# tgsstdio/BirdNest.Audio

Hardware: AMD Instinct MI355X
Metric: decoded PCM MSamples/s/GPU (bit-exact) + achieved HBM GB/s vs roofline (higher is better)
Workload: dtype int32; 1 GPU; C2: 1024-frame batches, 44.1 kHz/16-bit stereo, bs 4096, LPC-8, Rice partition order 4 -> FLACDecoder 16-bit LE interleaved PCM; frames_per_batch=1024, compressed_bytes_per_batch=10724000, pcm_bytes_per_batch=16777216, parallelism=corpus of 1 x 1024 batches partitioned per rank (shard.partition) x1

## Files before the change

birdnest/audio_amd/csrc/bnflac_kernels.hip:

```cpp
#include <hip/hip_runtime.h>
#include <stdint.h>
#include <stdlib.h>
#include <atomic>
#include <mutex>
#include <type_traits>

#include "bnflac_device.h"

#define DEV __device__ __forceinline__

__constant__ uint8_t g_crc8_tab[256];
__constant__ uint16_t g_crc16_tab[8][256];
__constant__ uint16_t g_crc16_xpow[40];
__device__ unsigned long long g_stats[16];
DEV uint64_t tnow(bool on) {
#ifndef BNFLAC_PHASE_TIMERS
    (void)on;
    return 0ull;
#endif
    if (!on) return 0ull;
    const uint64_t t = __builtin_amdgcn_s_memtime();
    asm volatile("s_waitcnt lgkmcnt(0)" ::: "memory");
    return t;
}
#define STAT(on, i) do { if (on) { if (__builtin_amdgcn_read_exec() && (threadIdx.x & 63) == (uint32_t)__builtin_ctzll(__builtin_amdgcn_read_exec())) atomicAdd(&g_stats[i], 1ull); } } while (0)

typedef __attribute__((address_space(3))) uint32_t lds_u32;
typedef __attribute__((address_space(3))) uint16_t lds_u16;
typedef __attribute__((address_space(3))) void lds_void;
typedef uint32_t u32x4 __attribute__((ext_vector_type(4)));
typedef __attribute__((address_space(3))) u32x4 lds_u32x4;
DEV void lds_st128(const void *a, u32x4 v) {
    asm volatile("ds_write_b128 %0, %1" ::"v"((uint32_t)(uintptr_t)a), "v"(v) : "memory");
}
DEV u32x4 lds_ld128(const void *a) {
    u32x4 v;
    asm volatile("ds_read_b128 %0, %1" : "=v"(v) : "v"((uint32_t)(uintptr_t)a) : "memory");
    return v;
}
DEV void lds_st128(const lds_u32x4 *a, u32x4 v) {
    asm volatile("ds_write_b128 %0, %1" ::"v"((uint32_t)(uintptr_t)a), "v"(v) : "memory");
}
DEV u32x4 lds_ld128(const lds_u32x4 *a) {
    u32x4 v;
    asm volatile("ds_read_b128 %0, %1" : "=v"(v) : "v"((uint32_t)(uintptr_t)a) : "memory");
    return v;
}
DEV void lds_st64(const void *a, uint64_t v) {
    asm volatile("ds_write_b64 %0, %1" ::"v"((uint32_t)(uintptr_t)a), "v"(v) : "memory");
}
DEV uint64_t lds_ld64(const void *a) {
    uint64_t v;
    asm volatile("ds_read_b64 %0, %1" : "=v"(v) : "v"((uint32_t)(uintptr_t)a) : "memory");
    return v;
}
typedef __attribute__((address_space(1))) const void gvoid;
DEV void gst128(uint64_t addr, u32x4 v) { *(__attribute__((address_space(1))) u32x4 *)addr = v; }

#define BNF_MODE_WREDO 0x4000u
#define BNF_MODE_SW 0x8000u
#define BNF_ABLATE_NO_SW 0x10000u
#define BNF_MODE_LIST 0x20000u
#define BNF_MODE_SEG 0x80000000u
#define BNF_MODE_NOST 0x40000u
#define BNF_MODE_STREDO 0x80000u
#define BNF_ABLATE_NO_W8SPLIT 0x100000u

#define RING_MAX 16
#define RING_LANE_DW 256

struct BR {
    const uint32_t *__restrict__ w;
    uint32_t nw;
    uint32_t nblk;
    lds_u32 *ring;
    lds_u32 *lring;
    uint32_t rdepth, wmask;
    uint32_t wi, s, hi, lo, nx;
    uint32_t vendw, iend;
    uint32_t iend_old;
    uint32_t ra, vlim;
    bool stats;
};

DEV void br_init(BR &b, const uint32_t *words, uint64_t nbytes, lds_u32 *ring, uint32_t lane, uint32_t rdepth) {
    b.rdepth = rdepth;
    b.wmask = 4u * rdepth - 1u;
    b.w = words;
    b.nblk = (uint32_t)((nbytes + 15u) >> 4);
    b.nw = b.nblk * 4u;
    b.ring = ring;
    b.lring = ring + lane * 4u;
    b.wi = 2;
    b.s = b.hi = b.lo = b.nx = 0;
    b.vendw = b.iend = 0;
    b.iend_old = 0;
    b.stats = false;
}

DEV void wait_vm() { asm volatile("s_waitcnt vmcnt(0)" ::: "memory"); }
template <int N> DEV void wait_vm_but() { asm volatile("s_waitcnt vmcnt(%0)" ::"i"(N) : "memory"); }
DEV void wait_vm_n(uint32_t n) {
    switch (__builtin_amdgcn_readfirstlane(min(n, 63u))) {
#define WVN(k) case k: asm volatile("s_waitcnt vmcnt(" #k ")" ::: "memory"); break;
#define WVN8(k) WVN(k) WVN(k + 1) WVN(k + 2) WVN(k + 3) WVN(k + 4) WVN(k + 5) WVN(k + 6) WVN(k + 7)
        WVN8(0) WVN8(8) WVN8(16) WVN8(24) WVN8(32) WVN8(40) WVN8(48) WVN8(56)
#undef WVN8
#undef WVN
    default: break;
    }
}
DEV void lds_sync() { asm volatile("s_waitcnt lgkmcnt(0)" ::: "memory"); }

DEV uint32_t gword(const BR &b, uint32_t w) { return (w < b.nw) ? b.w[w] : 0u; }
DEV uint32_t ring_off(const BR &b, uint32_t w) {
    return ((w & (b.wmask & ~3u)) << 6) + (w & 3u);
}
DEV uint32_t ring_word(const BR &b, uint32_t w) { return b.lring[ring_off(b, w)]; }
#define LDS_DMA_ALIGN __attribute__((aligned(1024)))
// ... 519 lines not shown

DEV uint32_t st_hmask(uint32_t h, uint32_t o) {
    return h <= o ? ~0u : (h >= o + 4u ? 0u : (~0u << (8u * (h - o))));
}
struct CrcZ {
    uint32_t r0, r1, px;
};
DEV void crcz_w(CrcZ &c, uint32_t le) {
    const uint32_t W = __builtin_bswap32(le);
    const uint32_t H = __builtin_amdgcn_alignbit(c.r1, c.r0, 28);
    const uint32_t n0 = W ^ H ^ (H << 4);
    c.r1 = c.r0 ^ (H >> 28);
    c.r0 = n0;
}
DEV void crcz_blk(CrcZ &c, uint4 v) {
    c.px ^= v.x ^ v.y ^ v.z ^ v.w;
    crcz_w(c, v.x);
    crcz_w(c, v.y);
    crcz_w(c, v.z);
    crcz_w(c, v.w);
}
struct CrcP {
    uint32_t s[15];
    uint32_t px;
    uint32_t wc;
};
DEV void crcp_init(CrcP &c) {
#pragma unroll
    for (int k = 0; k < 15; k++) c.s[k] = 0u;
    c.px = 0u;
    c.wc = ~0u;
}
DEV void crcp_fold(CrcP &c, const u32x4 (&v)[4]) {
    const uint32_t W[16] = {v[0].x, v[0].y, v[0].z, v[0].w, v[1].x, v[1].y, v[1].z, v[1].w,
                            v[2].x, v[2].y, v[2].z, v[2].w, v[3].x, v[3].y, v[3].z, v[3].w};
    c.px ^= W[0] ^ W[1] ^ W[2] ^ W[3] ^ W[4] ^ W[5] ^ W[6] ^ W[7] ^ W[8] ^ W[9] ^ W[10] ^ W[11] ^ W[12] ^ W[13] ^
            W[14] ^ W[15];
    const uint32_t r0 = c.s[13] ^ c.s[14] ^ W[15] ^ W[0], r1 = c.s[0] ^ c.s[13] ^ W[14] ^ W[0],
                   r2 = c.s[0] ^ c.s[1] ^ c.s[14] ^ W[13];
#pragma unroll
    for (int d = 14; d >= 3; d--) c.s[d] = c.s[d - 2] ^ c.s[d - 1] ^ W[15 - d];
    c.s[2] = r2;
    c.s[1] = r1;
    c.s[0] = r0;
    c.wc++;
}
DEV CrcZ crcp_z(const CrcP &c) {
    CrcZ z{0u, 0u, 0u};
#pragma unroll
    for (int k = 14; k >= 0; k--) crcz_w(z, c.s[k]);
    z.px = c.px;
    return z;
}
template <bool ALL = false, class C>
DEV void crcp_hook(C &c, const BR &b, uint32_t lane, uint32_t cl) {
    for (uint32_t it = 0; any_lane(c.wc < cl) && (ALL || it == 0u); it++) {
        if (c.wc < cl) {
            const uint32_t L = c.wc;
            u32x4 v[4];
            if (L + 2u >= (b.iend >> 2)) {
#pragma unroll
                for (uint32_t i = 0; i < 4; i++)
                    v[i] = lds_ld128((const lds_u32x4 *)(b.ring + (((L & 1u) * 4u + i) * RING_LANE_DW) + lane * 4u));
                lds_sync();
                crcp_fold(c, v);
            } else {
                const u32x4 *g = (const u32x4 *)((const uint8_t *)b.w + (uint64_t)L * 64u);
#pragma unroll
                for (uint32_t i = 0; i < 4; i++) v[i] = g[i];
                crcp_fold(c, v);
            }
        }
    }
}

#define CRC_LINES 4

DEV uint32_t byte_keep(int32_t lo, int32_t hi, int32_t w) {
    const int32_t a = min(max(lo - 4 * w, 0), 4), b = min(max(hi - 4 * w, 0), 4);
    const uint32_t mlo = a >= 4 ? 0u : (0xFFFFFFFFu << (8 * a));
    const uint32_t mhi = b >= 4 ? 0xFFFFFFFFu : ((1u << (8 * b)) - 1u);
    return mlo & mhi;
}
DEV bool crcz_zero(const CrcZ &c) {
    if (__builtin_popcount(c.px) & 1) return false;
    uint64_t v = ((uint64_t)(c.r1 & 0x0FFFFFFFu) << 32) | c.r0;
#pragma unroll
    for (int i = 0; i < 4; i++) {
        const uint64_t h = v >> 15;
        v = (v & 0x7FFFu) ^ h ^ (h << 1);
    }
    return v == 0;
}
DEV void crcz_line(CrcZ &c, uint4 (&v)[4], uint32_t h) {
    if (h) {
#pragma unroll
        for (int u = 0; u < 4; u++) {
            v[u].x &= st_hmask(h, 16u * u);
            v[u].y &= st_hmask(h, 16u * u + 4u);
            v[u].z &= st_hmask(h, 16u * u + 8u);
            v[u].w &= st_hmask(h, 16u * u + 12u);
        }
    }
#pragma unroll
    for (int u = 0; u < 4; u++) crcz_blk(c, v[u]);
}
template <int NL = CRC_LINES>
DEV bool st_crc16_ok(const uint8_t *__restrict__ bytes, uint64_t b0, uint64_t b1, CrcZ c = CrcZ{0u, 0u, 0u},
                     uint64_t from = 0) {
    const uint64_t p0 = max(b0 & ~(uint64_t)63u, from);
    const uint32_t h = p0 < b0 ? (uint32_t)(b0 & 63u) : 0u;
    const uint32_t nl = b1 > p0 ? (uint32_t)((b1 - p0) >> 6) : 0u;
    uint64_t p = p0;
    if (nl) {
        const uint4 *q = (const uint4 *)(bytes + p0);
        uint4 buf[NL][4];
#pragma unroll
        for (int d = 0; d < NL; d++)
#pragma unroll
            for (int u = 0; u < 4; u++) buf[d][u] = q[4u * min((uint32_t)d, nl - 1u) + u];
#pragma unroll
        for (int u = 0; u < 4; u++) {
// ... 590 lines not shown
    uint32_t incl = c;
    const uint32_t lane = threadIdx.x & 63;
    for (int o = 1; o < 64; o <<= 1) {
        uint32_t y = __shfl_up(incl, o);
        if (lane >= (unsigned)o) incl += y;
    }
    if (lane == 63) wtot[threadIdx.x >> 6] = incl;
    __syncthreads();
    uint32_t wpre = 0;
    for (uint32_t wv = 0; wv < (threadIdx.x >> 6); wv++) wpre += wtot[wv];
    uint32_t pos = block_offs[blockIdx.x] + wpre + incl - c;
    for (int i = 0; i < SCAN_BYTES_PER_THREAD; i++) {
        if (is_sync(d, n, base + i)) {
            if (pos < cap) out[pos] = base + i;
            pos++;
        }
    }
}

#define PARSE_RD 8
static_assert(PARSE_RD == 8, "pk_ra and the walk's pair steps (slot masks 0x3F3 / 0x1C0C, slot bits 10-12) assume an 8-slot ring");
template <int CPM>
DEV void parse_frame(const uint32_t *__restrict__ words, uint64_t nbytes, const uint64_t *__restrict__ frame_offs,
                     uint32_t nframes, const bnf_stream_params &sp, const uint64_t *__restrict__ out_sample_in,
                     uint64_t base_sample, bnf_frame_info *__restrict__ info, uint32_t ablate, lds_u32 *ring,
                     uint32_t f, uint32_t *__restrict__ crcp) {
    if (f >= nframes) return;
    bnf_frame_info fi;
    fi.status = BNF_ST_OK;
    fi.err = -1;
    fi.frame_off = frame_offs[f];
    fi.resume_bit = 0;
    fi.cached = -1;
    fi.blocksize = fi.sample_rate = fi.channels = fi.assignment = fi.bps = 0;
    fi.number_type = 0;
    fi.unparseable = 0;
    fi.number = 0;
    fi.out_sample = 0;
    fi.crc8 = fi.crc16_calc = fi.crc16_read = fi.crc_ok = 0;
    fi.flags = 0;
    fi.reserved = 0;
    uint32_t ss[8];
#pragma unroll
    for (int c = 0; c < 8; c++) ss[c] = 0;
    const uint64_t limit = nbytes * 8u;
    const uint64_t fbit = fi.frame_off * 8u;
    BR b;
    br_init(b, words, nbytes, ring, threadIdx.x, PARSE_RD);
    CrcP cp;
    crcp_init(cp);
    uint32_t st = parse_header(b, fbit, limit, sp, fi);
    if (st == BNF_ST_ERROR && br_pos(b) > limit) st = BNF_ST_TRUNC;
    if (CPM && crcp != nullptr && st == BNF_ST_OK && fi.channels == 2u && !(ablate & 16u)) {
        const uint32_t h = (uint32_t)(fi.frame_off & 63u);
        const u32x4 *g = (const u32x4 *)((const uint8_t *)words + (fi.frame_off & ~(uint64_t)63u));
        u32x4 v[4];
#pragma unroll
        for (uint32_t i = 0; i < 4; i++) {
            v[i] = g[i];
            v[i].x &= st_hmask(h, 16u * i);
            v[i].y &= st_hmask(h, 16u * i + 4u);
            v[i].z &= st_hmask(h, 16u * i + 8u);
            v[i].w &= st_hmask(h, 16u * i + 12u);
        }
        cp.wc = (uint32_t)(fi.frame_off >> 6);
        crcp_fold(cp, v);
    }
    if (st == BNF_ST_OK) {
        uint64_t sample;
        if (fi.number_type == 1) sample = fi.number;
        else if (sp.has_stream_info && sp.min_blocksize == sp.max_blocksize) sample = (uint64_t)sp.min_blocksize * fi.number;
        else sample = (uint64_t)fi.blocksize * fi.number;
        fi.out_sample = out_sample_in ? out_sample_in[f] : sample - base_sample;
        uint32_t maxorder = 0;
        bool raw = false;
        for (uint32_t ch = 0; ch < fi.channels; ch++) {
            const uint32_t here = (uint32_t)(br_pos(b) - fbit);
#pragma unroll
            for (int c = 0; c < 8; c++) ss[c] = (uint32_t)c == ch ? here : ss[c];
            if (ch + 1 == fi.channels) {
                const uint32_t x = br_peek(b) >> 24;
                if (!(x & 0x80u) && (x & 0x7Eu) >= 0x40u) maxorder = max(maxorder, ((x >> 1) & 31u) + 1u);
                raw = raw || (x & 0x7Eu) < 4u;
                break;
            }
            if (ablate & 16u) {
#pragma unroll
                for (int c = 0; c < 8; c++) ss[c] = (uint32_t)c == ch + 1 ? here : ss[c];
                continue;
            }
            SubHdr h;
            int32_t err = -1;
            uint32_t bps = sub_bps(fi, ch);
            st = parse_subframe_head<false>(b, bps, fi.blocksize, limit, h, nullptr, nullptr, err);
            if (st == BNF_ST_OK) {
                if (h.type == T_LPC) maxorder = max(maxorder, h.order);
                raw = raw || h.type == T_CONST || h.type == T_VERB;
                if (!(h.type == T_FIXED || h.type == T_LPC) || h.order > (fi.bps > 16u ? 12u : 8u)) cp.wc = ~0u;
                if (h.type == T_VERB) br_skip(b, (uint64_t)h.bps * fi.blocksize);
                else if (h.type == T_FIXED || h.type == T_LPC) st = skip_residual<CPM != 0>(b, h, fi.blocksize, limit, ablate, cp);
                if (st == BNF_ST_OK && br_pos(b) > limit) st = BNF_ST_TRUNC;
            }
            if (st == BNF_ST_ERROR && br_pos(b) > limit) st = BNF_ST_TRUNC;
            if (st != BNF_ST_OK) {
                if (st == BNF_ST_ERROR) {
                    fi.err = err;
                    fi.resume_bit = br_pos(b);
                }
                break;
            }
        }
        if (maxorder > 16) fi.flags |= BNF_FL_W32;
        else if (maxorder > 8 || (maxorder > 0 && fi.bps > 16)) fi.flags |= BNF_FL_W16;
        else if (fi.channels == 2 && fi.bps <= 16 && !raw) fi.flags |= BNF_FL_ST;
        if (maxorder > 0 && maxorder <= 12 && fi.channels == 2 && fi.bps > 16 && fi.bps <= 24 && !raw) fi.flags |= BNF_FL_SW;
    }
    fi.status = st;
#pragma unroll
// ... 1201 lines not shown
            if ((threadIdx.x & 63) >= (unsigned)o) incl += y;
        }
        if ((threadIdx.x & 63) == 63) wsum[threadIdx.x >> 6] = incl;
        __syncthreads();
        if (threadIdx.x == 0)
            for (int w = 1; w < 16; w++) wsum[w] += wsum[w - 1];
        __syncthreads();
        const uint64_t wprefix = (threadIdx.x >= 64) ? wsum[(threadIdx.x >> 6) - 1] : 0ull;
        if (i < n) v[i] = carry + wprefix + incl - x;
        __syncthreads();
        if (threadIdx.x == 1023) carry += wprefix + incl;
        __syncthreads();
    }
    if (threadIdx.x == 0) *total = carry;
}

__global__ void __launch_bounds__(256) k_chain_emit(const uint64_t *__restrict__ cand, uint32_t ncand,
                                                    const bnf_frame_info *__restrict__ info,
                                                    const uint32_t *__restrict__ mark, const uint32_t *__restrict__ pos,
                                                    const uint64_t *__restrict__ out_sample, bnf_stream_params sp,
                                                    uint64_t *__restrict__ d_offs, uint64_t *__restrict__ d_os,
                                                    bnf_frame_info *__restrict__ d_info, uint32_t cap,
                                                    uint32_t *__restrict__ nframes) {
    const uint32_t i = blockIdx.x * 256u + threadIdx.x;
    if (i >= ncand || !mark[i]) return;
    const uint32_t p = pos[i];
    if (p >= cap) return;
    const uint64_t os = out_sample[p];
    if (sp.has_stream_info && sp.total_samples > 0 && os >= sp.total_samples) {
        atomicMin(nframes, p);
        return;
    }
    d_offs[p] = cand[i];
    if (d_os) d_os[p] = os;
    if (d_info) {
        bnf_frame_info fi = info[i];
        fi.out_sample = os;
        d_info[p] = fi;
    }
}
#endif

#if BNF_TU == 3 || BNF_TU == 4 || BNF_TU == 7
#define ST_CHK 16
#define ST2_CHK 32
#define ST_RD 8

struct StCh {
    BR b;
    uint32_t cp[4];
    uint32_t q[8];
    int32_t sh;
    uint32_t k, km, k1, k32;
    uint32_t esc, left, pidx, nparts, psamples, plen, pesc, porder, order;
    uint32_t wasted;
    int32_t lim, mx, mn;
};

DEV uint32_t st_pk(int32_t lo, int32_t hi) { return __builtin_amdgcn_perm((uint32_t)hi, (uint32_t)lo, 0x05040100u); }
typedef short st_s2 __attribute__((ext_vector_type(2)));
DEV int32_t st_d2(uint32_t a, uint32_t b, int32_t acc) {
    return __builtin_amdgcn_sdot2(__builtin_bit_cast(st_s2, a), __builtin_bit_cast(st_s2, b), acc, false);
}
DEV int32_t st_d2z(uint32_t a, uint32_t b) {
    int32_t r;
    asm("v_dot2_i32_i16 %0, %1, %2, 0" : "=v"(r) : "v"(a), "v"(b));
    return r;
}

DEV bool st_setup(StCh &z, uint32_t bps, uint32_t bs, uint64_t limit) {
    SubHdr h;
    int32_t warm[8], coef[8], err = -1;
    const uint32_t st = parse_subframe_head<true, 8>(z.b, bps, bs, limit, h, warm, coef, err);
    if (st != BNF_ST_OK) return false;
    if (h.type != T_FIXED && h.type != T_LPC) return false;
    if (h.type == T_LPC && (h.order > 8 || h.path == P_WIDE)) return false;
    if (h.bps > 17) return false;
    int32_t c[8], w[8];
    bool in16 = true;
#pragma unroll
    for (int t = 0; t < 8; t++) {
        c[t] = 0;
        w[t] = ((uint32_t)t < h.order) ? warm[t] : 0;
        in16 = in16 && w[t] >= -32768 && w[t] <= 32767;
    }
    if (!in16) return false;
    z.sh = 0;
    z.lim = 0x7FFF;
    if (h.type == T_LPC) {
#pragma unroll
        for (int t = 0; t < 8; t++) c[t] = ((uint32_t)t < h.order) ? coef[t] : 0;
        if (h.path == P_MMX16) z.sh = ((uint32_t)h.shift >= 32u) ? 31 : h.shift;
        else z.sh = h.shift & 31;
    } else {
        const uint32_t o = h.order;
        c[0] = o == 1 ? 1 : o == 2 ? 2 : o == 3 ? 3 : o == 4 ? 4 : 0;
        c[1] = o == 2 ? -1 : o == 3 ? -3 : o == 4 ? -6 : 0;
        c[2] = o == 3 ? 1 : o == 4 ? 4 : 0;
        c[3] = o == 4 ? -1 : 0;
    }
#pragma unroll
    for (int k = 0; k < 4; k++) z.cp[k] = st_pk(c[2 * k], c[2 * k + 1]);
#pragma unroll
    for (int t = 0; t < 8; t++) z.q[t] = st_pk(w[t], t ? w[t - 1] : 0);
    z.order = h.order;
    z.wasted = h.wasted;
    z.porder = h.porder;
    z.nparts = 1u << h.porder;
    z.psamples = h.porder ? bs >> h.porder : bs - h.order;
    z.plen = h.rice2 ? 5u : 4u;
    z.pesc = h.rice2 ? 31u : 15u;
    z.left = 0;
    z.pidx = 0;
    z.esc = 0;
    z.k = 0;
    z.km = 31;
    z.k1 = 1;
    z.k32 = 32;
    z.mx = 0;
    z.mn = 0;
    return true;
}

template <class Z>
DEV void st_partition(Z &z) {
    const uint32_t kk = br_read(z.b, z.plen);
    z.left = (z.porder == 0 || z.pidx > 0) ? z.psamples : z.psamples - z.order;
    if (kk < z.pesc) {
        z.k = kk;
        z.esc = 0;
    } else {
        z.k = br_read(z.b, 5);
        z.esc = 1;
    }
    z.km = 31u - z.k;
    z.k1 = z.k + 1u;
    z.k32 = 32u - z.k;
    z.pidx++;
}

DEV void st_land(BR &b, uint32_t nst) {
    STAT(b.stats, 2);
    wait_vm_n(nst);
    b.vendw = b.iend * 4u;
    if (b.wi >= b.vendw) {
        br_refill(b);
        wait_vm();
        br_drained(b);
    }
}

DEV void st_adv(BR &b, uint32_t n, uint32_t nst) {
    const int32_t t = (int32_t)b.s - (int32_t)n;
    const bool c = t < 0;
    b.s = (uint32_t)t & 31u;
    b.hi = c ? b.lo : b.hi;
    b.lo = c ? __builtin_bswap32(b.nx) : b.lo;
    b.wi += c ? 1u : 0u;
    if (__builtin_expect(any_lane(b.wi >= b.vendw), 0)) st_land(b, nst);
    uint32_t off = ring_off(b, b.wi);
    asm volatile("" : "+v"(off) : "v"(b.lo));
    b.nx = b.lring[off];
}

template <class Z>
DEV int32_t st_rice(Z &z, uint64_t limit, uint32_t &trunc, uint32_t nst) {
    const uint32_t w = br_peek(z.b);
    const uint32_t q = ffbh(w);
    const bool slow = q >= z.k32;
    uint32_t u = (q << z.k) | __builtin_amdgcn_ubfe(w, z.km - q, z.k);
    const bool anyslow = any_lane(slow);
    st_adv(z.b, slow ? 0u : q + z.k1, nst);
    if (__builtin_expect(anyslow, 0)) {
        STAT(z.b.stats, 3);
        if (slow) {
            uint32_t qq;
            if (!br_unary(z.b, qq, limit)) trunc = 1;
            u = (qq << z.k) | br_read(z.b, z.k);
        }
    }
    return (int32_t)((u >> 1) ^ (0u - (u & 1u)));
}

template <class Z>
DEV int32_t st_next(Z &z, uint64_t limit, uint32_t &trunc, uint32_t nst) {
    while (z.left == 0) {
        if (z.pidx >= z.nparts) {
            trunc = 1;
            return 0;
        }
        st_partition(z);
    }
    z.left--;
    if (z.esc) return br_read_s(z.b, z.k);
    return st_rice(z, limit, trunc, nst);
}

template <int I>
DEV void st_dot2(const StCh &a, const StCh &b, int32_t &pa, int32_t &pb) {
#define Q_(z, j) z.q[(I + 8 - (j)) & 7]
    pa = st_d2(a.cp[3], Q_(a, 7), st_d2(a.cp[2], Q_(a, 5), st_d2(a.cp[1], Q_(a, 3), st_d2z(a.cp[0], Q_(a, 1)))));
    pb = st_d2(b.cp[3], Q_(b, 7), st_d2(b.cp[2], Q_(b, 5), st_d2(b.cp[1], Q_(b, 3), st_d2z(b.cp[0], Q_(b, 1)))));
#undef Q_
}

template <int T>
DEV void st_pre2(const StCh &a, const StCh &b, int32_t &pa, int32_t &pb) {
#define P_(z, j) z.q[(T + 8 - (j)) & 7]
    pa = st_d2(a.cp[3], P_(a, 6), st_d2(a.cp[2], P_(a, 4), st_d2z(a.cp[1], P_(a, 2))));
    pb = st_d2(b.cp[3], P_(b, 6), st_d2(b.cp[2], P_(b, 4), st_d2z(b.cp[1], P_(b, 2))));
#undef P_
}
DEV void st_fin2(const StCh &a, const StCh &b, uint32_t qa, uint32_t qb, int32_t prea, int32_t preb, int32_t &pa,
                 int32_t &pb) {
    pa = st_d2(a.cp[0], qa, prea);
    pb = st_d2(b.cp[0], qb, preb);
}

DEV void st_range(StCh &z, int32_t s0, int32_t s1) {
    z.mx = max(z.mx, max(s0, s1));
    z.mn = min(z.mn, min(s0, s1));
}

DEV void st_decor4(bool uni, uint32_t as_u, uint32_t as, int32_t (&L)[4], int32_t (&R)[4]) {
    const uint32_t a = uni ? as_u : as;
    if (a == 1) {
#pragma unroll
        for (int q = 0; q < 4; q++) R[q] = (int32_t)((uint32_t)L[q] - (uint32_t)R[q]);
    } else if (a == 2) {
#pragma unroll
        for (int q = 0; q < 4; q++) L[q] = (int32_t)((uint32_t)L[q] + (uint32_t)R[q]);
    } else if (a == 3) {
#pragma unroll
        for (int q = 0; q < 4; q++) {
            const uint32_t side = (uint32_t)R[q], mid = ((uint32_t)L[q] << 1) | (side & 1u);
            L[q] = (int32_t)(mid + side) >> 1;
            R[q] = (int32_t)(mid - side) >> 1;
        }
    }
}
// ... 196 lines not shown
    L[T & 3] = s0;
    R[T & 3] = s1;
    if ((T & 3) == 3) {
        if (AS < 0 && __builtin_expect(anyw, 0)) {
#pragma unroll
            for (int q = 0; q < 4; q++) {
                L[q] = (int32_t)((uint32_t)L[q] << z0.wasted);
                R[q] = (int32_t)((uint32_t)R[q] << z1.wasted);
            }
        }
        if (STG && AS >= 0) {
            pk[PO + (T >> 2)] = st_pack4<AS>(z0.q[(T + 6) & 7], z1.q[(T + 6) & 7], z0.q[T], z1.q[T]);
            return;
        }
        st_decor4t<AS>(as_uni, as_u, as, L, R);
        if (STG) {
            uint32_t w[4];
#pragma unroll
            for (int q = 0; q < 4; q++) w[q] = __builtin_amdgcn_perm((uint32_t)R[q], (uint32_t)L[q], 0x05040100u);
            pk[PO + (T >> 2)] = u32x4{w[0], w[1], w[2], w[3]};
        } else if (store) {
            st_emit4<FMT>(dst, nbase + (uint32_t)T - 3u, 4u, al, bs, L, R);
        }
    }
}

DEV uint32_t st_rice_pair(const StCh &z, uint32_t &ua, uint32_t &ub, bool &sl) {
    const uint32_t w = br_peek(z.b);
    const uint32_t qa = (uint32_t)__builtin_clz(w | 1u);
    const uint32_t la = qa + z.k1;
    const uint32_t w2 = w << (la & 31u);
    const uint32_t qb = (uint32_t)__builtin_clz(w2 | 1u);
    ua = (qa << z.k) | __builtin_amdgcn_ubfe(w, z.km - qa, z.k);
    ub = (qb << z.k) | __builtin_amdgcn_ubfe(w2, z.km - qb, z.k);
    const uint32_t n = la + qb + z.k1;
    sl = n > 32u;
    return sl ? 0u : n;
}
DEV void st_rare_pair(StCh &z, bool sl, bool ld, uint32_t &ua, uint32_t &ub, uint64_t limit, uint32_t &trunc,
                      uint32_t nst, uint32_t lane) {
    if (any_lane(ld)) {
        st_land(z.b, nst);
        if (z.b.wi + 1u >= z.b.vendw) {
            wait_vm();
            br_refill(z.b);
            wait_vm();
            br_drained(z.b);
        }
        st_next_word(z.b);
    }
    if (any_lane(sl)) {
        STAT(z.b.stats, 3);
        if (sl) {
            uint32_t qq;
            if (!br_unary(z.b, qq, limit)) trunc = 1;
            ua = (qq << z.k) | br_read(z.b, z.k);
            if (!br_unary(z.b, qq, limit)) trunc = 1;
            ub = (qq << z.k) | br_read(z.b, z.k);
        }
    }
    st_resync(z.b, lane);
}
template <int T, int FMT, int AS, int PO, int NPK>
DEV void st_fused_pair(StCh &z0, StCh &z1, int32_t (&L)[4], int32_t (&R)[4], uint64_t limit, uint32_t &trunc,
                       uint32_t nq, bool as_uni, uint32_t as_u, uint32_t as, uint8_t *dst, uint32_t nbase, bool al,
                       uint32_t bs, bool store, u32x4 (&pk)[NPK], int32_t &pre0, int32_t &pre1,
                       uint32_t lane, bool anyw) {
    static_assert((T & 1) == 0, "pairs start on even samples");
    constexpr bool STG = (FMT == BNF_OUT_FLACDECODER || FMT == BNF_OUT_FILEREADER);
    constexpr uint32_t spg = (FMT == BNF_OUT_INTERLEAVED32 || FMT == BNF_OUT_PLANAR32) ? 2u : 1u;
    const uint32_t nqt = nq + ((!STG && T >= 4 && store) ? spg : 0u);
    uint32_t u0a, u0b, u1a, u1b;
    bool sl0, sl1;
    const uint32_t n0 = st_rice_pair(z0, u0a, u0b, sl0), n1 = st_rice_pair(z1, u1a, u1b, sl1);
    const uint32_t laneb = lane << 4;
    st_adv_nc(z0.b, n0, laneb);
    st_adv_nc(z1.b, n1, laneb);
    constexpr bool CHK = (T & 2) == 0;
    const bool ld0 = CHK && z0.b.wi >= z0.b.vlim, ld1 = CHK && z1.b.wi >= z1.b.vlim;
    st_next_word(z0.b);
    st_next_word(z1.b);
    if (__builtin_expect(any_lane(sl0 || sl1 || ld0 || ld1), 0)) {
        st_rare_pair(z0, sl0, ld0, u0a, u0b, limit, trunc, nqt, lane);
        st_rare_pair(z1, sl1, ld1, u1a, u1b, limit, trunc, nqt, lane);
    }
    st_lpc_out<T, FMT, AS, PO, NPK>(z0, z1, u0a, u1a, L, R, as_uni, as_u, as, dst, nbase, al, bs, store, pk, pre0, pre1, anyw);
    st_lpc_out<T + 1, FMT, AS, PO, NPK>(z0, z1, u0b, u1b, L, R, as_uni, as_u, as, dst, nbase, al, bs, store, pk, pre0, pre1, anyw);
}

template <int T, int FMT>
DEV bool st_gen_step(StCh &z0, StCh &z1, int32_t (&L)[4], int32_t (&R)[4], uint64_t limit, uint32_t &trunc,
                     uint32_t nst, bool as_uni, uint32_t as_u, uint32_t as, uint8_t *dst, uint32_t n, bool valid,
                     bool al, uint32_t bs, bool store) {
    const bool v = valid && n < bs;
    int32_t s0 = 0, s1 = 0;
    if (v) {
        int32_t p0, p1;
        st_dot2<T>(z0, z1, p0, p1);
        if (n < z0.order) s0 = (int32_t)(int16_t)z0.q[T];
        else s0 = (int32_t)((uint32_t)st_next(z0, limit, trunc, nst) + (uint32_t)(p0 >> z0.sh));
        if (n < z1.order) s1 = (int32_t)(int16_t)z1.q[T];
        else s1 = (int32_t)((uint32_t)st_next(z1, limit, trunc, nst) + (uint32_t)(p1 >> z1.sh));
        st_range(z0, s0, s0);
        st_range(z1, s1, s1);
        z0.q[T] = __builtin_amdgcn_perm(z0.q[(T + 7) & 7], (uint32_t)s0, 0x05040100u);
        z1.q[T] = __builtin_amdgcn_perm(z1.q[(T + 7) & 7], (uint32_t)s1, 0x05040100u);
    }
    L[T & 3] = (int32_t)((uint32_t)s0 << z0.wasted);
    R[T & 3] = (int32_t)((uint32_t)s1 << z1.wasted);
    bool stored = false;
    if ((T & 3) == 3) {
// ... 13 lines not shown
                                                     const uint32_t *__restrict__ perm, uint32_t ablate,
                                                     const uint32_t *__restrict__ crcp) {
    constexpr bool STG = (FMT == BNF_OUT_FLACDECODER || FMT == BNF_OUT_FILEREADER);
    constexpr uint32_t ST_SPG = (FMT == BNF_OUT_INTERLEAVED32 || FMT == BNF_OUT_PLANAR32) ? 2u : 1u;
    __shared__ LDS_DMA_ALIGN uint32_t ring[2 * ST_RD * RING_LANE_DW + 1024];
    static_assert((ST_RD * RING_LANE_DW * 4) % 1024 == 0, "channel 1's ring base must stay 1 KiB aligned (LDS-DMA)");
    const uint32_t lane = threadIdx.x;
    const uint32_t slot = blockIdx.x * 64u + lane;
    const uint32_t f = (perm && slot < nframes) ? perm[slot] : slot;
    const uint64_t limit = nbytes * 8u;
    bnf_frame_info fi;
    const bool have = f < nframes;
    if (have) fi = info[f];
    const bool mine = have && fi.status == BNF_ST_OK && (fi.flags & BNF_FL_ST) && !(fi.flags & BNF_FL_REDO) &&
                      (!(ablate & BNF_MODE_WREDO) || (fi.flags & BNF_FL_WAVE_REDO));
    if (!__any(mine)) return;

    uint64_t stride = 0;
    bool ok = mine && fi.channels == 2 && chn_lanes >= 2;
    if (FMT == BNF_OUT_FLACDECODER) { stride = 4; ok = ok && fi.bps == 16 && sp.channels >= 2; }
    else if (FMT == BNF_OUT_FILEREADER) { stride = 4; ok = ok && sp.channels == 2 && sp.bps == 16; }
    else if (FMT == BNF_OUT_INTERLEAVED32) { stride = 8; ok = ok && sp.channels == 2; }
    else { stride = 4ull * sp.channels; ok = ok && sp.channels == 2; }
    const uint32_t bs = ok ? fi.blocksize : 0u;
    const uint64_t os = ok ? fi.out_sample : 0u;
    ok = ok && (os + bs) * stride <= out_bytes;
    uint8_t *dst = out + os * stride;
    const bool al = (((uintptr_t)dst) & 15u) == 0 && (FMT != BNF_OUT_PLANAR32 || (bs & 3u) == 0);

    StCh z0, z1;
    lds_u32 *ring0 = (lds_u32 *)ring, *ring1 = (lds_u32 *)ring + ST_RD * RING_LANE_DW;
    br_init(z0.b, words, nbytes, ring0, lane, ST_RD);
    br_init(z1.b, words, nbytes, ring1, lane, ST_RD);
    z0.b.stats = z1.b.stats = (ablate & 0x100u) != 0;
    STAT(z0.b.stats, 5);
    const bool tmon = z0.b.stats;
    const uint64_t t_start = tnow(tmon);
    uint64_t tm_dec = 0, tm_ref = 0, tm_pack = 0;
    if (ok) {
        br_seek(z0.b, fi.frame_off * 8u + fi.sub_start[0]);
        ok = st_setup(z0, sub_bps(fi, 0), bs, limit);
    }
    if (ok) {
        br_seek(z1.b, fi.frame_off * 8u + fi.sub_start[1]);
        ok = st_setup(z1, sub_bps(fi, 1), bs, limit);
    }
    const uint32_t as = ok ? fi.assignment : 0u;
    const bool anyw = any_lane(ok && (z0.wasted | z1.wasted) != 0u);
    const uint32_t as_u = __builtin_amdgcn_readfirstlane(as);
    const bool as_uni = !any_lane(ok && as != as_u);
    const int as_fix = (as_uni && !anyw && as_u <= 3u) ? (int)as_u : -1;
    lds_u32x4 *stg = (lds_u32x4 *)((lds_u32 *)ring + 2u * ST_RD * RING_LANE_DW);
    static_assert(sizeof(ring) >= (2 * ST_RD * RING_LANE_DW + 1024) * 4, "the flush's 4 KB staging tile lies past the two rings");

    uint32_t mybs = ok ? bs : 0u;
    for (int o = 32; o > 0; o >>= 1) mybs = max(mybs, (uint32_t)__shfl_xor(mybs, o));
    const uint32_t nchunks = (mybs + ST2_CHK - 1) / ST2_CHK;
    uint32_t trunc = 0;
    wait_vm();
    uint32_t nst = 0;
    const bool sto = !(ablate & 2u);
    auto refill = [&](bool want) {
        wait_vm_n(nst);
        z0.b.vendw = z0.b.iend * 4u;
        z1.b.vendw = z1.b.iend * 4u;
        st_refill_issue(z0.b, want);
        st_refill_issue(z1.b, want);
        nst = 0;
    };
    const uint64_t t_loop = tnow(tmon);
    for (uint32_t kc = 0; kc < nchunks; kc++) {
        const uint64_t ta = tnow(tmon);
        const uint32_t n0 = kc * ST2_CHK;
        const bool valid = ok && n0 < bs;
        bool fast = valid && n0 >= 8u && n0 + ST2_CHK <= bs && !(ablate & 12u);
        if (fast) {
            if (z0.left == 0 && z0.pidx < z0.nparts) st_partition(z0);
            if (z1.left == 0 && z1.pidx < z1.nparts) st_partition(z1);
            fast = !z0.esc && !z1.esc && z0.left >= ST2_CHK && z1.left >= ST2_CHK;
        }
        const bool fused = !any_lane(valid && !fast);
        u32x4 pk[4], pk0[4];
        if (fused) {
            if (valid) {
                STAT(z0.b.stats, 0);
                int32_t pre0, pre1;
                st_pre2<7>(z0, z1, pre0, pre1);
                st_resync(z0.b, lane);
                st_resync(z1.b, lane);
                auto chunk = [&](auto as_c) {
                    constexpr int AS = decltype(as_c)::value;
                    auto group = [&](auto g_c, uint32_t nb) {
                        constexpr uint32_t G = decltype(g_c)::value;
                        int32_t L[4], R[4];
                        const uint32_t nq = nst + (STG ? 0u : G * 2u * ST_SPG);
#define FPAIR(T) st_fused_pair<T, FMT, AS, 2 * G, 4>(z0, z1, L, R, limit, trunc, nq, as_uni, as_u, as, dst, nb, al, bs, sto, pk, pre0, pre1, lane, anyw)
                        FPAIR(0); FPAIR(2); FPAIR(4); FPAIR(6);
#undef FPAIR
                    };
#pragma unroll 1
                    for (uint32_t h = 0; h < 2; h++) {
                        const uint32_t nb = n0 + 16u * h;
                        group(std::integral_constant<uint32_t, 0>(), nb);
                        group(std::integral_constant<uint32_t, 1>(), nb + 8u);
                        if (h == 0) {
                            if (STG) {
#pragma unroll
                                for (int u = 0; u < 4; u++) pk0[u] = pk[u];
                            } else if (sto) {
                                nst += 4u * ST_SPG;
                            }
                            refill(true);
                            st_resync(z0.b, lane);
                            st_resync(z1.b, lane);
                        }
                    }
                };
                switch (as_fix) {
                case 0: chunk(std::integral_constant<int, 0>()); break;
                case 1: chunk(std::integral_constant<int, 1>()); break;
                case 2: chunk(std::integral_constant<int, 2>()); break;
                case 3: chunk(std::integral_constant<int, 3>()); break;
                default: chunk(std::integral_constant<int, -1>()); break;
                }
                z0.left -= ST2_CHK;
                z1.left -= ST2_CHK;
            } else {
                refill(false);
            }
            if (!STG && sto && any_lane(valid)) nst += 4u * ST_SPG;
        } else {
            STAT(z0.b.stats, 1);
#pragma unroll 1
            for (uint32_t g = 0; g < ST2_CHK / 8; g++) {
                int32_t L[4], R[4];
                const uint32_t nb = n0 + g * 8u;
                bool st0, st1;
#define GSTEP(T) st_gen_step<T, FMT>(z0, z1, L, R, limit, trunc, nst, as_uni, as_u, as, dst, nb + T, valid, al, bs, sto)
                GSTEP(0); GSTEP(1); GSTEP(2);
                st0 = GSTEP(3);
                if (any_lane(st0)) nst += 1u;
                GSTEP(4); GSTEP(5); GSTEP(6);
                st1 = GSTEP(7);
                if (any_lane(st1)) nst += 1u;
#undef GSTEP
                if (g == 1) refill(valid && nb + 8u < bs);
            }
        }
        const uint64_t tb = tnow(tmon);
        tm_dec += tb - ta;
        refill(valid && n0 + ST2_CHK < bs);
        const uint64_t tc = tnow(tmon);
        tm_ref += tc - tb;
        if (STG && fused) {
            uint64_t run = (valid && sto) ? (uint64_t)(uintptr_t)(dst + (uint64_t)n0 * 4u) : 0ull;
            if ((ablate & 0x10000000u) && run && out_bytes >= (1u << 20))
                run = (uint64_t)(uintptr_t)(out + (uint64_t)(blockIdx.x & 7u) * 65536u + lane * 1024u + ((n0 * 4u) & 1023u));
            const uint32_t rlo = (uint32_t)run, rhi = (uint32_t)(run >> 32);
            const uint32_t fr = lane & 31u, ul = lane & 7u;
#pragma unroll
            for (uint32_t r = 0; r < 2; r++) {
                if ((lane >> 5) == r) {
#pragma unroll
                    for (uint32_t u = 0; u < 8; u++) lds_st128(stg + fr * 8u + (u ^ (fr & 7u)), u < 4 ? pk0[u] : pk[u - 4]);
                }
                lds_sync();
                u32x4 v[4];
                uint64_t a[4];
#pragma unroll
                for (uint32_t i = 0; i < 4; i++) {
                    const uint32_t f = (lane >> 3) + 8u * i;
                    v[i] = lds_ld128(stg + f * 8u + (ul ^ (f & 7u)));
                    const uint32_t src = (32u * r + f) * 4u;
                    a[i] = ((uint64_t)(uint32_t)__builtin_amdgcn_ds_bpermute((int)src, (int)rhi) << 32) |
                           (uint32_t)__builtin_amdgcn_ds_bpermute((int)src, (int)rlo);
                }
                lds_sync();
#pragma unroll
                for (uint32_t i = 0; i < 4; i++) {
                    if (a[i]) gst128(a[i] + 16u * ul, v[i]);
                    if (any_lane(a[i] != 0)) nst += 1u;
                }
            }
        }
        tm_pack += tnow(tmon) - tc;
    }
    const uint64_t t_loopend = tnow(tmon);

    uint32_t crc_read = 0;
    uint64_t end_byte = 0, resume = 0;
    if (ok) {
        if (z0.mx > z0.lim || z0.mn < -z0.lim - 1 || z1.mx > z1.lim || z1.mn < -z1.lim - 1) ok = false;
        if (trunc) ok = false;
    }
    if (ok) {
        while (z1.pidx < z1.nparts) {
            const uint32_t kk = br_read(z1.b, z1.plen);
            if (kk >= z1.pesc) br_read(z1.b, 5);
            z1.pidx++;
        }
        const uint32_t padbits = (uint32_t)((8u - (br_pos(z1.b) & 7u)) & 7u);
        const uint32_t zp = br_read(z1.b, padbits);
        if (br_pos(z1.b) > limit || zp != 0) ok = false;
        end_byte = br_pos(z1.b) >> 3;
        crc_read = br_read(z1.b, 16);
        if (br_pos(z1.b) > limit) ok = false;
        resume = br_pos(z1.b);
    }
    uint32_t crc = crc_read;
    if (ok && !(ablate & 1u) && !st_crc16_frame((const uint8_t *)words, crcp, f, fi.frame_off, end_byte + 2u)) ok = false;
    if (ok && crc != crc_read) ok = false;
    if (ok) {
        info[f].resume_bit = resume;
        info[f].crc16_read = crc_read;
        info[f].crc16_calc = crc;
        info[f].crc_ok = 1u;
    } else if (mine) {
        info[f].flags = fi.flags | BNF_FL_REDO;
    }
    if (tmon && lane == 0) {
        const uint64_t t_end = tnow(tmon);
        atomicAdd(&g_stats[8], (unsigned long long)(t_loop - t_start));
        atomicAdd(&g_stats[9], (unsigned long long)tm_dec);
        atomicAdd(&g_stats[10], (unsigned long long)tm_ref);
        atomicAdd(&g_stats[11], (unsigned long long)tm_pack);
        atomicAdd(&g_stats[12], (unsigned long long)(t_end - t_loopend));
    }
}

#if BNF_TU == 7
#define SW_TAPS 12
struct StW {
    BR b;
    int32_t c[SW_TAPS];
    int32_t x[16];
    int32_t sh;
    uint32_t wide;
    uint32_t k, km, k1, k32;
    uint32_t esc, left, pidx, nparts, psamples, plen, pesc, porder, order;
    uint32_t wasted;
};

DEV bool sw_setup(StW &z, uint32_t bps, uint32_t bs, uint64_t limit) {
    SubHdr h;
    int32_t warm[SW_TAPS], coef[SW_TAPS], err = -1;
    const uint32_t st = parse_subframe_head<true, SW_TAPS>(z.b, bps, bs, limit, h, warm, coef, err);
    if (st != BNF_ST_OK) return false;
    if (h.type != T_FIXED && h.type != T_LPC) return false;
    if (h.order > SW_TAPS) return false;
    if (h.type == T_LPC && h.path == P_MMX16) return false;
    if (h.type == T_LPC && h.path == P_WIDE && ((uint32_t)h.shift & 0xFFu) >= 32u) return false;
#pragma unroll
    for (int t = 0; t < SW_TAPS; t++) z.c[t] = (h.type == T_LPC && (uint32_t)t < h.order) ? coef[t] : 0;
    if (h.type == T_FIXED) {
        const uint32_t o = h.order;
        z.c[0] = o == 1 ? 1 : o == 2 ? 2 : o == 3 ? 3 : o == 4 ? 4 : 0;
        z.c[1] = o == 2 ? -1 : o == 3 ? -3 : o == 4 ? -6 : 0;
        z.c[2] = o == 3 ? 1 : o == 4 ? 4 : 0;
        z.c[3] = o == 4 ? -1 : 0;
    }
#pragma unroll
    for (int t = 0; t < 16; t++) z.x[t] = (t < SW_TAPS && (uint32_t)t < h.order) ? warm[t < SW_TAPS ? t : 0] : 0;
    z.wide = (h.type == T_LPC && h.path == P_WIDE) ? 1u : 0u;
    z.sh = h.type == T_LPC ? (int32_t)((uint32_t)h.shift & (z.wide ? 0xFFu : 31u)) : 0;
    z.order = h.order;
    z.wasted = h.wasted;
    z.porder = h.porder;
    z.nparts = 1u << h.porder;
    z.psamples = h.porder ? bs >> h.porder : bs - h.order;
    z.plen = h.rice2 ? 5u : 4u;
    z.pesc = h.rice2 ? 31u : 15u;
// ... 1061 lines not shown
```

Baseline: 739,200 MSamples/s.

## Cut register pressure in stereo decode and add optional fused CRC folding

Drops nparts and pesc from the per-channel state and recomputes them from porder and plen. The pk0 staging registers are parked in LDS during the decode loop and reloaded before the flush. frame_off and flags are re-read from memory at the end instead of being held live, and the Rice parameter gets an asm barrier so it stays in a VGPR. An ablation-gated path folds the CRC16 inside the refill loop. It is off by default, so the default gains come from lower VGPR pressure, paid for with extra LDS traffic and reloads.

Result: no change. 741,100 MSamples/s (median of 2 runs) (+0.3%).

```diff
diff --git a/birdnest/audio_amd/csrc/bnflac_kernels.hip b/birdnest/audio_amd/csrc/bnflac_kernels.hip
--- a/birdnest/audio_amd/csrc/bnflac_kernels.hip
+++ b/birdnest/audio_amd/csrc/bnflac_kernels.hip
@@ -65,6 +65,7 @@
 #define BNF_MODE_NOST 0x40000u
 #define BNF_MODE_STREDO 0x80000u
 #define BNF_ABLATE_NO_W8SPLIT 0x100000u
+#define BNF_ABLATE_CRCFOLD 0x40000000u
 
 #define RING_MAX 16
 #define RING_LANE_DW 256
@@ -690,6 +691,22 @@
     z.px = c.px;
     return z;
 }
+DEV void crcp_line(u32x4 (&v)[4], const uint32_t *__restrict__ w, uint32_t nblk, uint32_t L) {
+    const u32x4 *g = (const u32x4 *)((const uint8_t *)w + (uint64_t)L * 64u);
+    const uint64_t blk = (uint64_t)L * 4u;
+#pragma unroll
+    for (uint32_t i = 0; i < 4; i++) v[i] = blk + i < nblk ? g[i] : u32x4{0u, 0u, 0u, 0u};
+}
+DEV void crcp_line_masked(u32x4 (&v)[4], const uint32_t *__restrict__ w, uint32_t nblk, uint32_t L, uint32_t h) {
+    crcp_line(v, w, nblk, L);
+#pragma unroll
+    for (uint32_t i = 0; i < 4; i++) {
+        v[i].x &= st_hmask(h, 16u * i);
+        v[i].y &= st_hmask(h, 16u * i + 4u);
+        v[i].z &= st_hmask(h, 16u * i + 8u);
+        v[i].w &= st_hmask(h, 16u * i + 12u);
+    }
+}
 template <bool ALL = false, class C>
 DEV void crcp_hook(C &c, const BR &b, uint32_t lane, uint32_t cl) {
     for (uint32_t it = 0; any_lane(c.wc < cl) && (ALL || it == 0u); it++) {
@@ -703,9 +720,7 @@
                 lds_sync();
                 crcp_fold(c, v);
             } else {
-                const u32x4 *g = (const u32x4 *)((const uint8_t *)b.w + (uint64_t)L * 64u);
-#pragma unroll
-                for (uint32_t i = 0; i < 4; i++) v[i] = g[i];
+                crcp_line(v, b.w, b.nblk, L);
                 crcp_fold(c, v);
             }
         }
@@ -1402,18 +1417,9 @@
     uint32_t st = parse_header(b, fbit, limit, sp, fi);
     if (st == BNF_ST_ERROR && br_pos(b) > limit) st = BNF_ST_TRUNC;
     if (CPM && crcp != nullptr && st == BNF_ST_OK && fi.channels == 2u && !(ablate & 16u)) {
-        const uint32_t h = (uint32_t)(fi.frame_off & 63u);
-        const u32x4 *g = (const u32x4 *)((const uint8_t *)words + (fi.frame_off & ~(uint64_t)63u));
         u32x4 v[4];
-#pragma unroll
-        for (uint32_t i = 0; i < 4; i++) {
-            v[i] = g[i];
-            v[i].x &= st_hmask(h, 16u * i);
-            v[i].y &= st_hmask(h, 16u * i + 4u);
-            v[i].z &= st_hmask(h, 16u * i + 8u);
-            v[i].w &= st_hmask(h, 16u * i + 12u);
-        }
         cp.wc = (uint32_t)(fi.frame_off >> 6);
+        crcp_line_masked(v, words, b.nblk, cp.wc, (uint32_t)(fi.frame_off & 63u));
         crcp_fold(cp, v);
     }
     if (st == BNF_ST_OK) {
@@ -2721,10 +2727,14 @@
     uint32_t q[8];
     int32_t sh;
     uint32_t k, km, k1, k32;
-    uint32_t esc, left, pidx, nparts, psamples, plen, pesc, porder, order;
+    uint32_t esc, left, pidx, psamples, plen, porder, order;
     uint32_t wasted;
     int32_t lim, mx, mn;
 };
+template <class Z> DEV uint32_t st_nparts(const Z &z) { return z.nparts; }
+template <class Z> DEV uint32_t st_pesc(const Z &z) { return z.pesc; }
+DEV uint32_t st_nparts(const StCh &z) { return 1u << z.porder; }
+DEV uint32_t st_pesc(const StCh &z) { return (1u << z.plen) - 1u; }
 
 DEV uint32_t st_pk(int32_t lo, int32_t hi) { return __builtin_amdgcn_perm((uint32_t)hi, (uint32_t)lo, 0x05040100u); }
 typedef short st_s2 __attribute__((ext_vector_type(2)));
@@ -2775,10 +2785,8 @@
     z.order = h.order;
     z.wasted = h.wasted;
     z.porder = h.porder;
-    z.nparts = 1u << h.porder;
     z.psamples = h.porder ? bs >> h.porder : bs - h.order;
     z.plen = h.rice2 ? 5u : 4u;
-    z.pesc = h.rice2 ? 31u : 15u;
     z.left = 0;
     z.pidx = 0;
     z.esc = 0;
@@ -2795,7 +2803,7 @@
 DEV void st_partition(Z &z) {
     const uint32_t kk = br_read(z.b, z.plen);
     z.left = (z.porder == 0 || z.pidx > 0) ? z.psamples : z.psamples - z.order;
-    if (kk < z.pesc) {
+    if (kk < st_pesc(z)) {
         z.k = kk;
         z.esc = 0;
     } else {
@@ -2854,7 +2862,7 @@
 template <class Z>
 DEV int32_t st_next(Z &z, uint64_t limit, uint32_t &trunc, uint32_t nst) {
     while (z.left == 0) {
-        if (z.pidx >= z.nparts) {
+        if (z.pidx >= st_nparts(z)) {
             trunc = 1;
             return 0;
         }
@@ -3157,11 +3165,12 @@
     if (any_lane(sl)) {
         STAT(z.b.stats, 3);
         if (sl) {
-            uint32_t qq;
+            uint32_t qq, k = z.k;
+            asm volatile("" : "+v"(k));
             if (!br_unary(z.b, qq, limit)) trunc = 1;
-            ua = (qq << z.k) | br_read(z.b, z.k);
+            ua = (qq << k) | br_read(z.b, k);
             if (!br_unary(z.b, qq, limit)) trunc = 1;
-            ub = (qq << z.k) | br_read(z.b, z.k);
+            ub = (qq << k) | br_read(z.b, k);
         }
     }
     st_resync(z.b, lane);
@@ -3281,6 +3290,33 @@
     const int as_fix = (as_uni && !anyw && as_u <= 3u) ? (int)as_u : -1;
     lds_u32x4 *stg = (lds_u32x4 *)((lds_u32 *)ring + 2u * ST_RD * RING_LANE_DW);
     static_assert(sizeof(ring) >= (2 * ST_RD * RING_LANE_DW + 1024) * 4, "the flush's 4 KB staging tile lies past the two rings");
+    const uint32_t park_x = ((lane >> 1) & 2u) | (((lane >> 1) ^ (lane >> 3)) & 1u);
+    const uint32_t park = (uint32_t)(uintptr_t)(stg + lane * 4u + park_x);
+
+    CrcP c1;
+    crcp_init(c1);
+    if (STG && ok && (ablate & BNF_ABLATE_CRCFOLD) && !(ablate & 1u)) {
+        bool seed = true;
+        if (crcp) {
+            const u32x4 v = *(const u32x4 *)(crcp + CRCP_WORDS * (uint64_t)f + 4u);
+            const u32x4 q = *(const u32x4 *)(crcp + CRCP_WORDS * (uint64_t)f);
+            if (v.x && v.z == (uint32_t)fi.frame_off) {
+                seed = false;
+            } else if (q.z && q.w == (uint32_t)fi.frame_off) {
+                c1.s[1] = __builtin_bswap32(q.y & 0x0FFFFFFFu);
+                c1.s[0] = __builtin_bswap32(q.x);
+                c1.px = q.y >> 31;
+                c1.wc = (uint32_t)(fi.frame_off >> 6) + q.z - 1u;
+                seed = false;
+            }
+        }
+        if (seed) {
+            u32x4 v[4];
+            c1.wc = (uint32_t)(fi.frame_off >> 6);
+            crcp_line_masked(v, words, z1.b.nblk, c1.wc, (uint32_t)(fi.frame_off & 63u));
+            crcp_fold(c1, v);
+        }
+    }
 
     uint32_t mybs = ok ? bs : 0u;
     for (int o = 32; o > 0; o >>= 1) mybs = max(mybs, (uint32_t)__shfl_xor(mybs, o));
@@ -3294,6 +3330,7 @@
         z0.b.vendw = z0.b.iend * 4u;
         z1.b.vendw = z1.b.iend * 4u;
         st_refill_issue(z0.b, want);
+        if (STG) crcp_hook(c1, z1.b, lane, z1.b.wi >> 4);
         st_refill_issue(z1.b, want);
         nst = 0;
     };
@@ -3304,12 +3341,12 @@
         const bool valid = ok && n0 < bs;
         bool fast = valid && n0 >= 8u && n0 + ST2_CHK <= bs && !(ablate & 12u);
         if (fast) {
-            if (z0.left == 0 && z0.pidx < z0.nparts) st_partition(z0);
-            if (z1.left == 0 && z1.pidx < z1.nparts) st_partition(z1);
+            if (z0.left == 0 && z0.pidx < st_nparts(z0)) st_partition(z0);
+            if (z1.left == 0 && z1.pidx < st_nparts(z1)) st_partition(z1);
             fast = !z0.esc && !z1.esc && z0.left >= ST2_CHK && z1.left >= ST2_CHK;
         }
         const bool fused = !any_lane(valid && !fast);
-        u32x4 pk[4], pk0[4];
+        u32x4 pk[4];
         if (fused) {
             if (valid) {
                 STAT(z0.b.stats, 0);
@@ -3335,7 +3372,7 @@
                         if (h == 0) {
                             if (STG) {
 #pragma unroll
-                                for (int u = 0; u < 4; u++) pk0[u] = pk[u];
+                                for (uint32_t u = 0; u < 4; u++) lds_st128((const lds_u32x4 *)(uintptr_t)(park ^ (u << 4)), pk[u]);
                             } else if (sto) {
                                 nst += 4u * ST_SPG;
                             }
@@ -3387,6 +3424,10 @@
                 run = (uint64_t)(uintptr_t)(out + (uint64_t)(blockIdx.x & 7u) * 65536u + lane * 1024u + ((n0 * 4u) & 1023u));
             const uint32_t rlo = (uint32_t)run, rhi = (uint32_t)(run >> 32);
             const uint32_t fr = lane & 31u, ul = lane & 7u;
+            u32x4 pk0[4];
+#pragma unroll
+            for (uint32_t u = 0; u < 4; u++) pk0[u] = lds_ld128((const lds_u32x4 *)(uintptr_t)(park ^ (u << 4)));
+            lds_sync();
 #pragma unroll
             for (uint32_t r = 0; r < 2; r++) {
                 if ((lane >> 5) == r) {
@@ -3423,9 +3464,9 @@
         if (trunc) ok = false;
     }
     if (ok) {
-        while (z1.pidx < z1.nparts) {
+        while (z1.pidx < st_nparts(z1)) {
             const uint32_t kk = br_read(z1.b, z1.plen);
-            if (kk >= z1.pesc) br_read(z1.b, 5);
+            if (kk >= st_pesc(z1)) br_read(z1.b, 5);
             z1.pidx++;
         }
         const uint32_t padbits = (uint32_t)((8u - (br_pos(z1.b) & 7u)) & 7u);
@@ -3437,7 +3478,27 @@
         resume = br_pos(z1.b);
     }
     uint32_t crc = crc_read;
-    if (ok && !(ablate & 1u) && !st_crc16_frame((const uint8_t *)words, crcp, f, fi.frame_off, end_byte + 2u)) ok = false;
+    uint64_t frame_off = 0;
+    uint32_t flags = 0;
+    if (mine) {
+        const bnf_frame_info *ri = info + f;
+        asm volatile("" : "+v"(ri));
+        frame_off = ri->frame_off;
+        flags = ri->flags;
+    }
+    if (STG && !(ablate & 1u)) {
+        const bool run = ok && c1.wc != ~0u;
+        if (any_lane(run)) {
+            if (!run) c1.wc = ~0u;
+            crcp_hook<true>(c1, z1.b, lane, (uint32_t)((end_byte + 2u) >> 6));
+        }
+        const uint64_t from = (uint64_t)c1.wc * 64u;
+        if (run && from <= end_byte + 2u) {
+            if (!st_crc16_ok((const uint8_t *)words, frame_off, end_byte + 2u, crcp_z(c1), from)) ok = false;
+        } else if (ok && !st_crc16_frame((const uint8_t *)words, crcp, f, frame_off, end_byte + 2u)) {
+            ok = false;
+        }
+    } else if (ok && !(ablate & 1u) && !st_crc16_frame((const uint8_t *)words, crcp, f, frame_off, end_byte + 2u)) ok = false;
     if (ok && crc != crc_read) ok = false;
     if (ok) {
         info[f].resume_bit = resume;
@@ -3445,7 +3506,7 @@
         info[f].crc16_calc = crc;
         info[f].crc_ok = 1u;
     } else if (mine) {
-        info[f].flags = fi.flags | BNF_FL_REDO;
+        info[f].flags = flags | BNF_FL_REDO;
     }
     if (tmon && lane == 0) {
         const uint64_t t_end = tnow(tmon);
```
